# danping/CoSLAM

Measured on AMD Instinct MI355X. Metric: frames/sec for track+local-BA loop, 8 cams 640x480 x 2000 feats (one frame = all 8 cameras), higher is better.
Workload: dtype f32 (KLT, f16 pyramid storage) + f64 (pose, BA)

## Files before the change

coslam_amd/csrc/poseupdate.hip:

```cpp
#include <atomic>
#include <cstdlib>
#include <vector>

#include "cs_common.h"
#include "project_dev.h"
#include "history_view.h"
#include "register_rows_dev.h"
#include "small_ops.h"

#pragma clang fp contract(off)

namespace {

constexpr int PU_MAX_CAMS = 16;
constexpr int PU_MAX_HIST = 512;
constexpr int PU_MAX_STORE = 1 << 16;
constexpr int PU_LPS = 8;

struct PuArgs {
    int nCams, N, nMap, cam0, nCamsRun;
    int gateBlocks, dynBlocksPerCam;
    const int* pointFeat;
    const double* R;
    const double* t;
// ... 302 lines not shown
        double M[3], cov[9];
#pragma unroll
        for (int q = 0; q < 3; ++q) M[q] = A.M[3 * (size_t)p + q];
#pragma unroll
        for (int q = 0; q < 9; ++q) cov[q] = A.cov[9 * (size_t)p + q];
        const int f1 = C.trackSpan[s], f2 = C.trackSpan[N + s];
        const int len = f1 >= 0 ? f2 - f1 + 1 : 0;
        const int depth = len < A.nHist ? len : A.nHist;
        cut = len > A.nHist;
        for (int j = r; j < depth && !fail && !cut; j += MG_LPC) {
            const double* R = mg_pose + 12 * j;
            const double* t = R + 9;
            const int rs = (A.head - j + H) % H;
            const double mx = hXY[(size_t)rs * 2 * N + s], my = hXY[(size_t)rs * 2 * N + N + s];
            fail = mg_term_fails(C.K, R, t, M, cov, A.sigma, mx, my);
        }
    }
    const unsigned long long b = __builtin_amdgcn_ballot_w64(fail);
    if (live && r == 0) {
        const bool anyFail = ((b >> (MG_LPC * g)) & ((1ull << MG_LPC) - 1ull)) != 0ull;
        A.out[(size_t)p * A.nCams + c] = s < 0 ? 255 : (cut ? 2 : (anyFail ? 0 : 1));
    }
}


struct MgCache {
    int slot1;
    int f1;
    int upto;
    int ok;
    double M[3];
    int epoch;
    int pad;
};
static_assert(sizeof(MgCache) == 48, "cs_register_mergability_cache_bytes");
struct MgRunCore {
    MgCore a;
    int W, count, curFrame;
    double tolPix;
    MgCache* cache;
    int epoch, fromMin;
    int* counts;
    const int* list;
    int nList;
    const int* flags;
};
struct MgRunArgs : MgRunCore {
    cs_poseupdate_cam cam[PU_MAX_CAMS];
};
constexpr int MG_GAP_MAX = 2 * MG_LPC;
struct MgMiss {
    int p, s, start, end;
};
template <int NT>
__device__ __forceinline__ void mg_running_rows(const MgRunCore& B, const cs_poseupdate_cam* cams, const int* list, int nList, int c, int bx,
                                                double* mg_pose, MgMiss* missList, int& nMiss) {
    const MgCore& A = B.a;
    const int tid = threadIdx.x, N = A.N, H = A.H, W = B.W;
    if (list && (int)(bx * (NT / MG_LPC)) < nList && list[bx * (NT / MG_LPC)] < 0) return;
    const cs_poseupdate_cam& C = cams[c];
    const double* hR = A.histR + (size_t)c * H * 9;
    const double* hT = A.histT + (size_t)c * H * 3;
    const double* hXY = A.histXY + (size_t)c * H * 2 * N;
    for (int q = tid; q < W * 12; q += NT) {
        const int j = q / 12, e = q - 12 * j, rs = (A.head - j + H) % H;
        mg_pose[q] = e < 9 ? hR[(size_t)rs * 9 + e] : hT[(size_t)rs * 3 + (e - 9)];
    }
    if (tid == 0) nMiss = 0;
    __syncthreads();
    const int lane = tid & 63, r = lane % MG_LPC, g = lane / MG_LPC;
    const unsigned long long gmask = ((1ull << MG_LPC) - 1ull) << (MG_LPC * g);
    const int jj = (bx * NT + tid) / MG_LPC;
    const int p = list ? (jj < nList ? list[jj] : -1) : (jj < A.P ? jj : -1);
    const bool live = p >= 0 && p < A.P;
    int s = live ? A.slot[(size_t)p * A.nCams + c] : -1;
    bool skipped = false;
    if (s >= 0 && B.flags && !(B.flags[(size_t)p * A.nCams + c] & 1)) skipped = true, s = -2;
    bool failW = false, cut = false, tailOK = true, hit = false, listed = false;
    int nTerms = 0;
    if (s >= 0) {
        double M[3], cov[9];
#pragma unroll
        for (int q = 0; q < 3; ++q) M[q] = A.M[3 * (size_t)p + q];
#pragma unroll
        for (int q = 0; q < 9; ++q) cov[q] = A.cov[9 * (size_t)p + q];
        const int f1 = C.trackSpan[s], f2 = C.trackSpan[N + s];
        const int len = f1 >= 0 ? f2 - f1 + 1 : 0;
        const int depth = len < W ? len : W;
        for (int j = r; j < depth && !failW; j += MG_LPC) {
            const double* R = mg_pose + 12 * j;
            const double* t = R + 9;
            const int rs = (A.head - j + H) % H;
            const double mx = hXY[(size_t)rs * 2 * N + s], my = hXY[(size_t)rs * 2 * N + N + s];
            failW = mg_term_fails(C.K, R, t, M, cov, A.sigma, mx, my);
        }
        failW = (__builtin_amdgcn_ballot_w64(failW) & gmask) != 0ull;
        const int end = B.curFrame - W;
        if (len > W) {
            MgCache* E = B.cache + (size_t)p * A.nCams + c;
            const MgCache e = *E;
            const PuProj q0 = pu_project(C.K, mg_pose, mg_pose + 9, M), q1 = pu_project(C.K, mg_pose, mg_pose + 9, e.M);
            const double du = q0.u / q0.w - q1.u / q1.w, dv = q0.v / q0.w - q1.v / q1.w;
            hit = e.slot1 == s + 1 && e.f1 == f1 && e.upto >= f1 - 1 && e.upto <= end && q0.w > 0 && q1.w > 0 &&
                  du * du + dv * dv <= B.tolPix * B.tolPix && (e.epoch == B.epoch || e.upto < B.fromMin);
            const int start = hit ? e.upto + 1 : f1;
            tailOK = hit ? e.ok != 0 : true;
// ... 42 lines not shown
            w.M[0] = M[0], w.M[1] = M[1], w.M[2] = M[2], w.epoch = B.epoch, w.pad = 0;
            B.cache[(size_t)p * A.nCams + c] = w;
        }
    }
    if (live && r == 0 && !listed) A.out[(size_t)p * A.nCams + c] = s == -1 ? 255 : (skipped ? 0 : (cut ? 2 : (failW || !tailOK ? 0 : 1)));
    __syncthreads();
    const int wv = tid >> 6, nM = nMiss;
    for (int k = wv; k < nM; k += NT / 64) {
        const MgMiss m = missList[k];
        double M[3], cov[9];
#pragma unroll
        for (int q = 0; q < 3; ++q) M[q] = A.M[3 * (size_t)m.p + q];
#pragma unroll
        for (int q = 0; q < 9; ++q) cov[q] = A.cov[9 * (size_t)m.p + q];
        bool ok = true;
        for (int f = m.start; f <= m.end && ok; f += 64) {
            bool fail = false;
            const int ff = f + lane;
            if (ff <= m.end) {
                const int j = B.curFrame - ff, rs = ((A.head - j) % H + H) % H;
                double Rt[12];
#pragma unroll
                for (int q = 0; q < 9; ++q) Rt[q] = hR[(size_t)rs * 9 + q];
#pragma unroll
                for (int q = 0; q < 3; ++q) Rt[9 + q] = hT[(size_t)rs * 3 + q];
                const double mx = hXY[(size_t)rs * 2 * N + m.s], my = hXY[(size_t)rs * 2 * N + N + m.s];
                fail = mg_term_fails(C.K, Rt, Rt + 9, M, cov, A.sigma, mx, my);
                ++nTerms;
            }
            if (__builtin_amdgcn_ballot_w64(fail)) ok = false;
        }
        if (lane == 0) {
            MgCache* E = B.cache + (size_t)m.p * A.nCams + c;
            const bool fresh = m.start == C.trackSpan[m.s];
            MgCache w;
            w.slot1 = m.s + 1, w.f1 = C.trackSpan[m.s], w.upto = m.end, w.ok = ok ? 1 : 0;
            w.M[0] = fresh ? M[0] : E->M[0], w.M[1] = fresh ? M[1] : E->M[1], w.M[2] = fresh ? M[2] : E->M[2], w.epoch = B.epoch, w.pad = 0;
            *E = w;
            A.out[(size_t)m.p * A.nCams + c] = ok ? 1 : 0;
        }
    }
    if (B.counts) {
        const unsigned long long bh = __builtin_amdgcn_ballot_w64(hit && r == 0), bw = __builtin_amdgcn_ballot_w64(listed && !hit && r == 0),
                                 bc = __builtin_amdgcn_ballot_w64(cut && r == 0);
        int terms = nTerms;
#pragma unroll
        for (int o = 32; o > 0; o >>= 1) terms += __shfl_xor(terms, o, 64);
        if (lane == 0) {
            if (bh) atomicAdd(B.counts, __popcll(bh));
            if (bw) atomicAdd(B.counts + 1, __popcll(bw));
            if (bc) atomicAdd(B.counts + 2, __popcll(bc));
            if (terms) atomicAdd(B.counts + 3, terms);
        }
    }
}
__global__ __launch_bounds__(256) void k_register_mergability_running(MgRunArgs B) {
    extern __shared__ double mg_pose[];
    __shared__ MgMiss missList[256 / MG_LPC];
    __shared__ int nMiss;
    CS_POSE_STREAM_PRIO();
    mg_running_rows<256>(B, B.cam, B.list, B.nList, B.a.cam0 + blockIdx.y, blockIdx.x, mg_pose, missList, nMiss);
}


struct UpArgs {
    int nCams, N, nMap, H, head, nHist, firstKeyFrame;
    const int* pointFeat;
    const int* lastFrame;
    const unsigned char* isCurrent;
    const double* histXY;
    const double* histR;
    const double* histT;
    double* mapPts;
    double* mapCov;
    const unsigned char* mapFlags;
    double sigma;
    int* counts;
    const double* cen;
    int refine;
    const unsigned char* select;
    const int4* featRef;
    const unsigned char* refStatic;
    const int4* segPool;
    int segCap, curFrame, stored;
    cs_poseupdate_cam cam[PU_MAX_CAMS];
};
constexpr int UP_LPP = 64;

static_assert(UP_LPP == 64 && PU_MAX_CAMS <= UP_LPP, "the covariance tail broadcasts from lane = camera of the point's own wave");

struct UpNormalEq {
    double N[6], g[3];
};
__device__ __forceinline__ void up_add_view(UpNormalEq& E, const double* __restrict__ iK, const double* __restrict__ R,
                                            const double* __restrict__ t, double mx, double my) {
    const double w = (iK[6] * mx + iK[7] * my) + iK[8];
    const double x = ((iK[0] * mx + iK[1] * my) + iK[2]) / w, y = ((iK[3] * mx + iK[4] * my) + iK[5]) / w;
    const double a0[3] = {R[0] - x * R[6], R[1] - x * R[7], R[2] - x * R[8]}, a1[3] = {R[3] - y * R[6], R[4] - y * R[7], R[5] - y * R[8]};
    const double b0 = x * t[2] - t[0], b1 = y * t[2] - t[1];
    E.N[0] = E.N[0] + (a0[0] * a0[0] + a1[0] * a1[0]);
    E.N[1] = E.N[1] + (a0[0] * a0[1] + a1[0] * a1[1]);
    E.N[2] = E.N[2] + (a0[0] * a0[2] + a1[0] * a1[2]);
    E.N[3] = E.N[3] + (a0[1] * a0[1] + a1[1] * a1[1]);
    E.N[4] = E.N[4] + (a0[1] * a0[2] + a1[1] * a1[2]);
    E.N[5] = E.N[5] + (a0[2] * a0[2] + a1[2] * a1[2]);
#pragma unroll
// ... 2013 lines not shown
        }
    }
}

extern "C" int cs_feat_ref_advance_refine_dev(cs_track_history* h, void* hip_stream, const cs_poseupdate_cam* cams, int nMap, const int* d_pointFeat,
                                              int curFrame, cs_feat_ref* d_featRef, unsigned char* d_refStatic, int* d_counts, const int* d_list,
                                              int nList, int advanceAll, unsigned char* d_select, int clearSelect, double* d_mapPts,
                                              double* d_mapCov, double pixelErrVar) {
    if (!h || !cams || nMap < 1 || nList < 1 || !d_pointFeat || !d_featRef || !d_list || !d_select || !d_mapPts || !d_mapCov) {
        cs_set_error("cs_feat_ref_advance_refine_dev: bad arguments");
        return CS_ERR_INVALID;
    }
    if (h->count < 1 || curFrame != h->lastFrame) {
        cs_set_error("cs_feat_ref_advance_refine_dev: the history's newest entry must be frame %d (it holds %d frame(s), the newest %d)", curFrame,
                     h->count, h->lastFrame);
        return CS_ERR_INVALID;
    }
    ArArgs A;
    memset((void*)&A, 0, sizeof(A));
    A.nMap = nMap, A.featRef = (const int4*)d_featRef, A.mapPts = d_mapPts, A.mapCov = d_mapCov, A.sigma = pixelErrVar;
    A.refine = 1, A.select = d_select, A.selectW = d_select, A.clearSelect = clearSelect ? 1 : 0;
    A.segPool = h->segPool, A.segCap = h->segCap, A.curFrame = h->lastFrame, A.stored = h->count < h->H ? h->count : h->H;
    A.nCams = h->nCams, A.N = h->N, A.H = h->H, A.head = h->head, A.nHist = hist_walk(h);
    A.histXY = h->xy, A.histR = h->R, A.histT = h->t, A.cen = h->cen;
    A.F.nCams = h->nCams, A.F.N = h->N, A.F.nMap = nMap, A.F.curFrame = curFrame, A.F.segCap = h->segCap;
    A.F.pointFeat = d_pointFeat, A.F.featRef = (int4*)d_featRef, A.F.refStatic = d_refStatic, A.F.segPool = h->segPool, A.F.segCount = h->segCount;
    A.F.counts = d_counts;
    A.list = d_list, A.nList = nList, A.advAll = advanceAll ? 1 : 0;
    CS_HIP(hipSetDevice(h->device));
    hipStream_t s = (hipStream_t)hip_stream;
    if (nMap > h->aliveCap) {
        if (h->alive) CS_HIP(hipFree(h->alive));
        h->alive = nullptr, h->aliveCap = 0;
        CS_HIP(hipMalloc((void**)&h->alive, (size_t)nMap));
        CS_HIP(hipMemsetAsync(h->alive, 1, (size_t)nMap, s));
        h->aliveCap = nMap;
    }
    A.F.alive = h->alive;
    for (int c = 0; c < h->nCams; ++c) {
        if (!cams[c].K || !cams[c].iK || !cams[c].trackSpan) {
            cs_set_error("cs_feat_ref_advance_refine_dev: null pointer in camera %d (K, iK, trackSpan are read)", c);
            return CS_ERR_INVALID;
        }
        A.cam[c] = cams[c];
    }
    hist_centres(h, s);
    A.blocksA = ((advanceAll ? nMap : nList) + 255) / 256;
    hipLaunchKernelGGL(k_advance_refine, dim3(A.blocksA + (nList + 3) / 4), dim3(256), 0, s, A);
    CS_HIP(hipGetLastError());
    return CS_OK;
}

constexpr int RR_THREADS = 256;
struct RrArgs {
    int nRounds, W, H;
    int* lists;
    int* rvCounts;
    cs_register_pass pass;
    cs_register_cam rcam[RG_MAX_CAMS];
    MgRunCore mg;
    RvArgs rv;
    ArArgs ar;
};
static_assert(sizeof(RrArgs) <= 4096, "k_revisit_rounds: the arguments must fit the kernel-argument segment");
template <int MC>
__global__ __launch_bounds__(RR_THREADS) void k_revisit_rounds(RrArgs A) {
    extern __shared__ double rr_pose[];
    __shared__ MgMiss missList[RR_THREADS / MG_LPC];
    __shared__ int nMiss;
    __shared__ int sCnt[RR_THREADS / 64][5];
    if (rd_ld(A.rvCounts) == 0) return;
    CS_POSE_STREAM_PRIO();
    const int tid = threadIdx.x, lane = tid & 63, wave = tid >> 6, C = A.rv.nCams, cap = A.rv.cap, N = A.rv.N;
    const cs_register_pass& Q = A.pass;
    int cnt[5] = {0, 0, 0, 0, 0};
    for (int r = 0; r < A.nRounds; ++r) {
        const int listed = rd_ld(A.rvCounts + r);
        if (listed == 0) break;
        const int n = listed < cap ? listed : cap;
        const int* list = A.lists + (size_t)r * cap;
        for (int k = wave; k < n * C; k += RR_THREADS / 64) {
            const int row = k / C, c = k - row * C, p = list[row];
            if (p < 0) continue;
            const cs_register_cam& Cm = A.rcam[c];
            const size_t o = (size_t)p * C + c;
            int outSlot = -1, outFlags = 0;
            double m0 = 0, m1 = 0, var[4] = {0, 0, 0, 0}, ivar[4] = {0, 0, 0, 0}, outDist = 0;
            Proj q;
            if (rg_pair_begin(Q, Cm, o, p, A.W, A.H, q, m0, m1, var, ivar, outSlot)) {
                double dMin;
                int iMin;
                rg_pair_scan_wave(Cm, N, lane, m0, m1, ivar, dMin, iMin);
                rg_pair_finish(Q, Cm, p, N, q, m0, m1, dMin, iMin, outSlot, outFlags, outDist);
            }
            if (lane == 0) rg_pair_store(Q, o, outSlot, outFlags, outDist, m0, m1, var);
        }
        __syncthreads();
        const int nB = (n * MG_LPC + RR_THREADS - 1) / RR_THREADS;
        for (int c = 0; c < C; ++c)
            for (int bx = 0; bx < nB; ++bx) {
                mg_running_rows<RR_THREADS>(A.mg, A.ar.cam, list, cap, c, bx, rr_pose, missList, nMiss);
                __syncthreads();
            }
        {
            const bool more = r + 1 < A.nRounds;
            const RvRound Rd{list, A.rvCounts + r, more ? A.lists + (size_t)(r + 1) * cap : nullptr, more ? A.rvCounts + r + 1 : nullptr};
            if (n <= RR_THREADS) {
                rv_decide_rows<MC>(A.rv, Rd);
            } else {
                int* rowCode = (int*)(rr_pose + 12 * (size_t)A.mg.W);
                rv_decide_rows_looped<MC, RR_THREADS>(A.rv, Rd, n, rowCode, rowCode + MC * RV_MAX_ROWS);
            }
        }
        __syncthreads();
        for (int j = tid; j < n; j += RR_THREADS) {
            const int m = list[j];
            if (m >= 0 && m < A.ar.nMap && !A.ar.select[m]) fr_advance_row(A.ar.F, A.ar.cam, m, cnt);
        }
        __syncthreads();
        for (int j = wave; j < n; j += RR_THREADS / 64) {
            const int m = list[j];
            if (m >= 0 && m < A.ar.nMap && A.ar.select[m]) ar_refine_row(A.ar, m, lane, cnt);
        }
        __syncthreads();
    }
    if (A.ar.F.counts) {
#pragma unroll
        for (int k = 0; k < 5; ++k) {
            int v = cnt[k];
#pragma unroll
            for (int o = 32; o > 0; o >>= 1) v += __shfl_xor(v, o, 64);
            if (lane == 0) sCnt[wave][k] = v;
        }
        __syncthreads();
        if (tid < 5) {
            int v = 0;
            for (int w = 0; w < RR_THREADS / 64; ++w) v += sCnt[w][tid];
            if (v) atomicAdd(A.ar.F.counts + tid, v);
        }
    }
}
template <int MC>
static int rr_dynamic_lds_limit(int device, size_t* out) {
    static std::atomic<long long> last{-1};
    const long long c = last.load(std::memory_order_acquire);
    if (c >= 0 && (int)(c >> 32) == device) {
        *out = (size_t)(c & 0xffffffffll);
        return CS_OK;
    }
    hipFuncAttributes fa;
    CS_HIP(hipFuncGetAttributes(&fa, (const void*)k_revisit_rounds<MC>));
    constexpr size_t total = MC == 8 ? 65536 : 163840;
    if (fa.sharedSizeBytes >= total) {
        cs_set_error("k_revisit_rounds<%d>: %zu B of static LDS", MC, (size_t)fa.sharedSizeBytes);
        return CS_ERR_INVALID;
    }
    const size_t dyn = total - fa.sharedSizeBytes;
    if (total > 65536) CS_HIP(hipFuncSetAttribute((const void*)k_revisit_rounds<MC>, hipFuncAttributeMaxDynamicSharedMemorySize, (int)dyn));
    if (device >= 0) last.store(((long long)device << 32) | (long long)dyn, std::memory_order_release);
    *out = dyn;
    return CS_OK;
}

extern "C" int cs_register_revisit_rounds_dev(cs_track_history* h, void* hip_stream, const cs_register_cam* regCams, const cs_poseupdate_cam* cams,
                                              int W, int H, const cs_register_pass* pass, int nMap, int curFrame, int mapBase, int kinds,
                                              double* d_mapPts, double* d_mapCov, double pixelErrVar, double tolPix, void* d_mergeCache,
                                              unsigned char* d_mergeable, int* d_rvLists, int* d_rvCounts, int cap, int nRounds, int* d_visitLoop,
                                              int* d_nextLoop, const unsigned char* d_mapFlags, int* d_pointFeat, int* const* d_slot2map,
                                              unsigned char* d_attached, unsigned char* d_regOut, void* d_decideScratch, const int* d_curList,
                                              const int* d_curCount, int curCap, int* d_rvCnt, cs_feat_ref* d_featRef, unsigned char* d_refStatic,
                                              int* d_frefCounts) {
    if (!h || !regCams || !cams || !pass) {
        cs_set_error("cs_register_revisit_rounds_dev: bad arguments (null history, cameras or pass)");
        return CS_ERR_INVALID;
    }
    const int nCams = h->nCams, N = h->N;
    const cs_register_pass& q = *pass;
// ... 18 lines not shown
        cs_set_error("cs_register_revisit_rounds_dev: the history's newest entry must be frame %d (it holds %d frame(s), the newest %d)", curFrame,
                     h->count, h->lastFrame);
        return CS_ERR_INVALID;
    }
    RrArgs A;
    memset((void*)&A, 0, sizeof(A));
    for (int c = 0; c < nCams; ++c) {
        const cs_register_cam& rc = regCams[c];
        if (!rc.K || !rc.R || !rc.t || !rc.xy || !rc.state || !rc.slot2map) {
            cs_set_error("cs_register_revisit_rounds_dev: null pointer in search camera %d", c);
            return CS_ERR_INVALID;
        }
        if (!cams[c].K || !cams[c].iK || !cams[c].trackSpan) {
            cs_set_error("cs_register_revisit_rounds_dev: null pointer in camera %d (K, iK, trackSpan are read)", c);
            return CS_ERR_INVALID;
        }
        if (!d_slot2map[c]) {
            cs_set_error("cs_register_revisit_rounds_dev: null slot2map of camera %d", c);
            return CS_ERR_INVALID;
        }
        A.rcam[c] = rc;
    }
    A.nRounds = nRounds, A.W = W, A.H = H, A.lists = d_rvLists, A.rvCounts = d_rvCounts;
    A.pass = q;
    A.pass.P = cap, A.pass.list = nullptr;
    MgCore& G = A.mg.a;
    G.cam0 = 0, G.nCams = nCams, G.N = N, G.P = nMap, G.H = h->H, G.head = h->head, G.nHist = hist_walk(h);
    G.sigma = pixelErrVar, G.M = d_mapPts, G.cov = d_mapCov, G.slot = q.slot, G.out = d_mergeable;
    G.histXY = h->xy, G.histR = h->R, G.histT = h->t;
    A.mg.W = hist_walk(h), A.mg.count = h->count, A.mg.curFrame = h->lastFrame, A.mg.epoch = h->tailEpoch, A.mg.fromMin = h->tailFromMin;
    A.mg.tolPix = tolPix, A.mg.cache = (MgCache*)d_mergeCache, A.mg.counts = nullptr, A.mg.flags = q.flags;
    RvArgs& V = A.rv;
    V.nCams = nCams, V.N = N, V.P = nMap, V.cap = cap, V.mapBase = mapBase, V.kinds = kinds, V.nextLoop = d_nextLoop, V.visitLoop = d_visitLoop;
    V.slot = q.slot, V.flags = q.flags, V.mergeable = d_mergeable, V.mapFlags = d_mapFlags, V.pointFeat = d_pointFeat;
    for (int c = 0; c < nCams; ++c) V.slot2map[c] = d_slot2map[c];
    V.attached = d_attached, V.regOut = d_regOut, V.curList = d_curList, V.curCount = d_curCount, V.curCap = curCap, V.counts = d_rvCnt;
    V.nextLoopW = d_nextLoop, V.overflow = d_rvCounts + nRounds;
    V.debug = cs_debug_get(CS_DBG_MERGE_PRINT) == 1;
    int* scr = (int*)d_decideScratch + (size_t)nCams * nMap + nMap;
    for (int k = 0; k < 3; ++k) V.owner[k] = scr, scr += (size_t)nCams * N;
    ArArgs& R = A.ar;
    R.nMap = nMap, R.featRef = (const int4*)d_featRef, R.mapPts = d_mapPts, R.mapCov = d_mapCov, R.sigma = pixelErrVar;
    R.refine = 1, R.select = d_regOut, R.selectW = d_regOut, R.clearSelect = 1;
    R.segPool = h->segPool, R.segCap = h->segCap, R.curFrame = h->lastFrame, R.stored = h->count < h->H ? h->count : h->H;
    R.nCams = nCams, R.N = N, R.H = h->H, R.head = h->head, R.nHist = hist_walk(h);
    R.histXY = h->xy, R.histR = h->R, R.histT = h->t, R.cen = h->cen;
    R.F.nCams = nCams, R.F.N = N, R.F.nMap = nMap, R.F.curFrame = curFrame, R.F.segCap = h->segCap;
    R.F.pointFeat = d_pointFeat, R.F.featRef = (int4*)d_featRef, R.F.refStatic = d_refStatic, R.F.segPool = h->segPool, R.F.segCount = h->segCount;
    R.F.counts = d_frefCounts;
    for (int c = 0; c < nCams; ++c) R.cam[c] = cams[c];
    CS_HIP(hipSetDevice(h->device));
    hipStream_t s = (hipStream_t)hip_stream;
    const int MC = nCams <= 8 ? 8 : RD_MAX_CAMS;
    const size_t lds = sizeof(double) * 12 * (size_t)A.mg.W + (cap > RR_THREADS ? sizeof(int) * (size_t)(MC + 1) * RV_MAX_ROWS : 0);
    size_t ldsMax = 0;
    if (const int rc = MC == 8 ? rr_dynamic_lds_limit<8>(h->device, &ldsMax) : rr_dynamic_lds_limit<RD_MAX_CAMS>(h->device, &ldsMax)) return rc;
    if (lds > ldsMax) {
        cs_set_error("cs_register_revisit_rounds_dev: %zu B of LDS (a history window of %d frames, lists of %d rows, %d cameras) where the "
                     "launch may carry %zu", lds, A.mg.W, cap, nCams, ldsMax);
        return CS_ERR_INVALID;
    }
    if (nMap > h->aliveCap) {
        if (h->alive) CS_HIP(hipFree(h->alive));
        h->alive = nullptr, h->aliveCap = 0;
        CS_HIP(hipMalloc((void**)&h->alive, (size_t)nMap));
        CS_HIP(hipMemsetAsync(h->alive, 1, (size_t)nMap, s));
        h->aliveCap = nMap;
    }
    R.F.alive = h->alive;
    hist_centres(h, s);
    if (MC == 8)
        hipLaunchKernelGGL(k_revisit_rounds<8>, dim3(1), dim3(RR_THREADS), lds, s, A);
    else
        hipLaunchKernelGGL(k_revisit_rounds<RD_MAX_CAMS>, dim3(1), dim3(RR_THREADS), lds, s, A);
    CS_HIP(hipGetLastError());
    return CS_OK;
}

extern "C" int cs_track_history_segments(const cs_track_history* h, cs_feat_seg** d_pool, int* cap, int** d_count) {
    if (!h) {
        cs_set_error("cs_track_history_segments: null handle");
        return CS_ERR_INVALID;
    }
    if (d_pool) *d_pool = (cs_feat_seg*)h->segPool;
    if (cap) *cap = h->segCap;
    if (d_count) *d_count = h->segCount;
    return CS_OK;
}

extern "C" int cs_track_history_segment_counts(const cs_track_history* h, int* counts) {
    if (!h || !counts) {
        cs_set_error("cs_track_history_segment_counts: bad arguments");
        return CS_ERR_INVALID;
    }
    CS_HIP(hipSetDevice(h->device));
    CS_HIP(hipMemcpy(counts, h->segCount, sizeof(int) * h->nCams, hipMemcpyDeviceToHost));
    return CS_OK;
}

extern "C" int cs_track_history_load_segments(cs_track_history* h, const cs_feat_seg* segs, int n) {
    if (!h || n < 0 || n > h->segCap || (n > 0 && !segs)) {
        cs_set_error("cs_track_history_load_segments: bad arguments (at most %d segments per camera)", h ? h->segCap : 0);
        return CS_ERR_INVALID;
    }
    CS_HIP(hipSetDevice(h->device));
    std::vector<int> cnt(h->nCams, n);
    for (int c = 0; c < h->nCams && n > 0; ++c)
        CS_HIP(hipMemcpy(h->segPool + (size_t)c * h->segCap, segs + (size_t)c * n, sizeof(int4) * n, hipMemcpyHostToDevice));
    CS_HIP(hipMemcpy(h->segCount, cnt.data(), sizeof(int) * h->nCams, hipMemcpyHostToDevice));
    return CS_OK;
}

extern "C" int cs_track_history_download_segments(const cs_track_history* h, cs_feat_seg* segs, int n) {
    if (!h || !segs || n < 0 || n > h->segCap) {
        cs_set_error("cs_track_history_download_segments: bad arguments (at most %d segments per camera)", h ? h->segCap : 0);
        return CS_ERR_INVALID;
    }
    CS_HIP(hipSetDevice(h->device));
    for (int c = 0; c < h->nCams && n > 0; ++c)
        CS_HIP(hipMemcpy(segs + (size_t)c * n, h->segPool + (size_t)c * h->segCap, sizeof(int4) * n, hipMemcpyDeviceToHost));
    return CS_OK;
}

namespace {
template <class Args>
void up_set_refs(Args& A, const cs_track_history* h) {
    A.segPool = h->segPool, A.segCap = h->segCap, A.curFrame = h->lastFrame, A.stored = h->count < h->H ? h->count : h->H;
// ... 297 lines not shown
```

coslam_amd/csrc/register_rows_dev.h:

```cpp
#pragma once

#include "cs_common.h"

#include <cfloat>

#pragma clang fp contract(off)

namespace {

constexpr int RG_MAX_CAMS = 16;

struct Proj {
    double u, v, w;
    double KR[9];
};

__device__ __forceinline__ void projection_cov(const Proj& q, const double* __restrict__ cov, double sigma, double var[4]) {
    const double ww = q.w * q.w;
    double J[6], JC[6];
#pragma unroll
    for (int j = 0; j < 3; ++j) {
        J[j] = (q.KR[j] * q.w - q.u * q.KR[6 + j]) / ww;
        J[3 + j] = (q.KR[3 + j] * q.w - q.v * q.KR[6 + j]) / ww;
    }
// ... 30 lines not shown
    const double X = ((R[0] * M[0] + R[1] * M[1]) + R[2] * M[2]) + t[0];
    const double Y = ((R[3] * M[0] + R[4] * M[1]) + R[5] * M[2]) + t[1];
    const double Z = ((R[6] * M[0] + R[7] * M[1]) + R[8] * M[2]) + t[2];
    if (Z < 0.0) {
        outSlot = -2;
        return false;
    }
    q.u = (K[0] * X + K[1] * Y) + K[2] * Z;
    q.v = (K[3] * X + K[4] * Y) + K[5] * Z;
    q.w = (K[6] * X + K[7] * Y) + K[8] * Z;
    m0 = q.u / q.w;
    m1 = q.v / q.w;
    if (m0 < 0 || m0 >= (double)W || m1 < 0 || m1 >= (double)H) {
        outSlot = -3;
        return false;
    }
#pragma unroll
    for (int i = 0; i < 3; ++i)
#pragma unroll
        for (int j = 0; j < 3; ++j) q.KR[3 * i + j] = (K[3 * i] * R[j] + K[3 * i + 1] * R[3 + j]) + K[3 * i + 2] * R[6 + j];
    projection_cov(q, Q.cov + 9 * (size_t)p, Q.sigmaSearch, var);
    mat22_inv(var, ivar);
    const bool dynPt = Q.mapFlags && (Q.mapFlags[p] & (CS_MAP_DYNAMIC | CS_MAP_FALSE | CS_MAP_UNCERTAIN)) == CS_MAP_DYNAMIC;
    const double sc = 1 / (dynPt ? Q.maxDistDynamic : Q.maxDist);
#pragma unroll
    for (int k = 0; k < 4; ++k) ivar[k] = ivar[k] * sc;
    return true;
}
__device__ __forceinline__ void rg_pair_finish(const cs_register_pass& Q, const cs_register_cam& C, int p, int N, const Proj& q, double m0,
                                               double m1, double dMin, int iMin, int& outSlot, int& outFlags, double& outDist) {
    if (iMin == 0x7fffffff) {
        outSlot = -4;
        return;
    }
    outSlot = iMin;
    outDist = dMin;
    if (C.slot2map[iMin] < 0) outFlags |= 1;
    if (C.isDynamic ? C.isDynamic[iMin] != 0 : (C.isStatic && C.isStatic[iMin] == 0)) outFlags |= 2;
    double v2[4], iv[4];
    projection_cov(q, Q.cov + 9 * (size_t)p, Q.sigmaMerge, v2);
    mat22_inv(v2, iv);
    if (!(maha_dist2(m0, m1, C.xy[iMin], C.xy[N + iMin], iv) > 1.0)) outFlags |= 4;
}
__device__ __forceinline__ void rg_pair_store(const cs_register_pass& Q, size_t o, int outSlot, int outFlags, double outDist, double m0, double m1,
                                              const double var[4]) {
    Q.slot[o] = outSlot;
    Q.flags[o] = outFlags;
    Q.dist[o] = outDist;
    Q.m[2 * o] = m0;
    Q.m[2 * o + 1] = m1;
#pragma unroll
    for (int k = 0; k < 4; ++k) Q.var[4 * o + k] = var[k];
}
__device__ __forceinline__ void rg_pair_scan_wave(const cs_register_cam& C, int N, int lane, double m0, double m1, const double ivar[4],
                                                  double& dMin, int& iMin) {
    dMin = DBL_MAX, iMin = 0x7fffffff;
    const double* __restrict__ xs = C.xy;
    const double* __restrict__ ys = C.xy + N;
    const int* __restrict__ st = C.state;
    for (int i = lane; i < N; i += 64) {
        const int s = st[i];
        if (s == 0 || s == 1) {
            const double d = maha_dist2(m0, m1, xs[i], ys[i], ivar);
            if (d < dMin) dMin = d, iMin = i;
        }
    }
#pragma unroll
    for (int off = 32; off > 0; off >>= 1) {
        const double d2 = __shfl_xor(dMin, off, 64);
        const int i2 = __shfl_xor(iMin, off, 64);
        if (d2 < dMin || (d2 == dMin && i2 < iMin)) dMin = d2, iMin = i2;
    }
}

constexpr int RD_MAX_CAMS = 16;
constexpr int RD_INIT_MAPPED = 1 << 29, RD_CAN_MERGE = 1 << 28, RD_FEAT = (1 << 28) - 1;
constexpr int RD_INF = 0x7fffffff;
__device__ __forceinline__ int rd_ld(const int* p) { return __hip_atomic_load(p, __ATOMIC_RELAXED, __HIP_MEMORY_SCOPE_AGENT); }
__device__ __forceinline__ void rd_st(int* p, int v) { __hip_atomic_store(p, v, __ATOMIC_RELAXED, __HIP_MEMORY_SCOPE_AGENT); }

struct RvArgs {
    int nCams, N, P, cap, mapBase, kinds;
    const int* list;
    const int* nextLoop;
    int* visitLoop;
    const int* slot;
    const int* flags;
    const unsigned char* mergeable;
    const unsigned char* mapFlags;
    int* pointFeat;
    int* slot2map[RD_MAX_CAMS];
    unsigned char* attached;
    unsigned char* regOut;
    int* owner[3];
    const int* curList;
    const int* curCount;
    int curCap;
    int* counts;
    const int* listCount;
    int* nextList;
    int* nextCount;
    int* nextLoopW;
    int* overflow;
    int debug;
};
constexpr int RV_MAX_ROWS = 1024;
struct RvRound {
    const int* list;
    const int* listCount;
    int* nextList;
    int* nextCount;
};
__device__ __forceinline__ RvRound rv_round_of(const RvArgs& A) { return RvRound{A.list, A.listCount, A.nextList, A.nextCount}; }
__device__ __forceinline__ int* rv_owner(const RvArgs& A, int k) {
    const int r = k % 3;
    return r == 0 ? A.owner[0] : (r == 1 ? A.owner[1] : A.owner[2]);
}
template <int MC>
__device__ __forceinline__ void rv_row_build(const RvArgs& A, int p, int (&code)[MC], int& base, int& nConf) {
    const int C = A.nCams;
    int kind = -1;
    base = -1;
#pragma unroll
    for (int i = 0; i < MC; ++i) code[i] = -1;
    int pfv[MC], slv[MC], flv[MC], own[MC];
    unsigned char mgv[MC];
// ... 99 lines not shown
            }
        }
    }
    if (reg) {
        ++nReg;
        const int last = A.nextLoop[p];
        A.regOut[p] = 1, A.visitLoop[p] = last;
        if (Rd.nextList) {
            int b = -1;
            for (int c = C - 1; c > last; --c)
                if (A.pointFeat[(size_t)p * C + c] >= 0) b = c;
            if (b >= 0) {
                const int q = atomicAdd(Rd.nextCount, 1);
                if (q < A.cap) Rd.nextList[q] = p, A.nextLoopW[p] = b;
                else if (A.overflow) atomicAdd(A.overflow, 1);
            }
        }
    }
}
template <int MC>
__device__ __forceinline__ void rv_conflicts_of(const RvArgs& A, int q, const int (&qs)[MC], const RvAttached& S, int nA, int& nConf) {
    const int C = A.nCams;
    bool any = false;
    for (int a = 0; a < nA && !any; ++a) {
        const int i = S.cam[a], sl = S.sl[a];
#pragma unroll
        for (int t = 0; t < MC; ++t) any |= t == i && qs[t] == sl;
    }
    if (!any) return;
    int qp[MC];
    unsigned qatt = 0;
#pragma unroll
    for (int i = 0; i < MC; ++i) {
        const size_t kq = (size_t)q * C + (i < C ? i : 0);
        qp[i] = A.pointFeat[kq];
        if (i < C && A.attached[kq]) qatt |= 1u << i;
    }
    int lq = -1;
#pragma unroll
    for (int i = MC - 1; i >= 0; --i)
        if (i < C && qp[i] >= 0 && !((qatt >> i) & 1u)) lq = i;
    if (lq < 0) return;
    for (int a = 0; a < nA; ++a) {
        const int i = S.cam[a], sl = S.sl[a];
        int qsi = -1, qpi = 0;
#pragma unroll
        for (int t = 0; t < MC; ++t)
            if (t == i) qsi = qs[t], qpi = qp[t];
        if (qsi != sl || qpi >= 0) continue;
        if ((lq * A.P + q) * C + i <= S.key[a]) continue;
        if ((qatt >> (i + 1)) != 0u) ++nConf;
    }
}
template <int MC>
__device__ __forceinline__ void rv_decide_rows(const RvArgs& A, const RvRound& Rd) {
    __shared__ int sChanged;
    __shared__ RvAttached sAtt;
    const int j = threadIdx.x, C = A.nCams;
    const long long tD0 = A.debug ? wall_clock64() : 0;
    long long tD1 = 0, tD2 = 0, tD3 = 0;
    const int p = j < A.cap ? Rd.list[j] : -1;
    int code[MC], base = -1, nConf = 0;
    if (j == 0) sAtt.n = 0;
    const int nCurPre = *A.curCount < A.curCap ? *A.curCount : A.curCap;
    int preQ[2], preS[2][MC];
#pragma unroll
    for (int u = 0; u < 2; ++u) {
        const int e = j + u * (int)blockDim.x;
        preQ[u] = e < nCurPre ? A.curList[e] : -1;
        if (preQ[u] >= A.P) preQ[u] = -1;
#pragma unroll
        for (int i = 0; i < MC; ++i) preS[u][i] = preQ[u] >= 0 ? A.slot[(size_t)preQ[u] * C + (i < C ? i : 0)] : -1;
    }
    rv_row_build<MC>(A, p, code, base, nConf);
    __syncthreads();
    if (A.debug) tD1 = wall_clock64();
    int k = 0;
    const int* fin = A.owner[0];
    bool settled = false;
    for (; k < 32; ++k) {
        const int* prev = rv_owner(A, k);
        int* next = rv_owner(A, k + 1);
        int* clear = rv_owner(A, k + 2);
        if (j == 0) sChanged = 0;
        rv_row_clear<MC>(code, base, clear);
        __syncthreads();
        rv_row_claim<MC>(code, base, prev, next);
        __syncthreads();
        if (rv_row_changed<MC>(code, base, prev, next)) sChanged = 1;
        __syncthreads();
        fin = next;
        const int chg = sChanged;
        __syncthreads();
        if (!chg) {
            settled = true;
            break;
        }
    }
    if (A.debug) tD2 = wall_clock64();
    int nAtt = 0, nReg = 0;
    rv_row_attach<MC>(A, Rd, p, code, base, fin, sAtt, nAtt, nReg);
    __syncthreads();
    if (A.debug) tD3 = wall_clock64();
    const int nA = sAtt.n < 256 ? sAtt.n : 256;
    if (nA > 0) {
        const int nCur = nCurPre;
        for (int e = j, u = 0; e < nCur; e += (int)blockDim.x, ++u) {
            const int q = u == 0 ? preQ[0] : (u == 1 ? preQ[1] : A.curList[e]);
            if (q < 0 || q >= A.P) continue;
            int qs[MC];
#pragma unroll
            for (int i = 0; i < MC; ++i) qs[i] = u == 0 ? preS[0][i] : (u == 1 ? preS[1][i] : A.slot[(size_t)q * C + (i < C ? i : 0)]);
            rv_conflicts_of<MC>(A, q, qs, sAtt, nA, nConf);
        }
    }
    if (A.debug && j == 0)
        printf("k_revisit_decide: rows %d; build %lld us, %d sweeps %lld us, attach %lld us (%d attached), scan %lld us\n", Rd.listCount ? *Rd.listCount : -1,
               (tD1 - tD0) / 100, k + 1, (tD2 - tD1) / 100, (tD3 - tD2) / 100, nA, (wall_clock64() - tD3) / 100);
    if (A.counts) {
        if (nAtt) atomicAdd(A.counts, nAtt);
        if (nReg) atomicAdd(A.counts + 1, nReg);
        if (nConf) atomicAdd(A.counts + 2, nConf);
        if (j == 0 && !settled) atomicAdd(A.counts + 3, 1);
    }
}
template <int MC, int NT>
__device__ __forceinline__ void rv_decide_rows_looped(const RvArgs& A, const RvRound& Rd, int n, int* rowCode, int* rowBase) {
    __shared__ int sChanged;
    __shared__ RvAttached sAtt;
    const int tid = threadIdx.x, C = A.nCams;
    int code[MC], base, nConf = 0;
    if (tid == 0) sAtt.n = 0;
    for (int j = tid; j < n; j += NT) {
        rv_row_build<MC>(A, Rd.list[j], code, base, nConf);
        rowBase[j] = base;
#pragma unroll
        for (int i = 0; i < MC; ++i) rowCode[i * RV_MAX_ROWS + j] = code[i];
    }
    __syncthreads();
    int k = 0;
    const int* fin = A.owner[0];
    bool settled = false;
    for (; k < 32; ++k) {
        const int* prev = rv_owner(A, k);
        int* next = rv_owner(A, k + 1);
        int* clear = rv_owner(A, k + 2);
        if (tid == 0) sChanged = 0;
        for (int j = tid; j < n; j += NT) {
#pragma unroll
            for (int i = 0; i < MC; ++i) code[i] = rowCode[i * RV_MAX_ROWS + j];
            rv_row_clear<MC>(code, rowBase[j], clear);
        }
        __syncthreads();
        for (int j = tid; j < n; j += NT) {
#pragma unroll
            for (int i = 0; i < MC; ++i) code[i] = rowCode[i * RV_MAX_ROWS + j];
            rv_row_claim<MC>(code, rowBase[j], prev, next);
        }
        __syncthreads();
        int ch = 0;
        for (int j = tid; j < n; j += NT) {
#pragma unroll
            for (int i = 0; i < MC; ++i) code[i] = rowCode[i * RV_MAX_ROWS + j];
            ch |= rv_row_changed<MC>(code, rowBase[j], prev, next);
        }
        if (ch) sChanged = 1;
        __syncthreads();
        fin = next;
        const int chg = sChanged;
        __syncthreads();
        if (!chg) {
            settled = true;
            break;
        }
    }
    int nAtt = 0, nReg = 0;
    for (int j = tid; j < n; j += NT) {
#pragma unroll
        for (int i = 0; i < MC; ++i) code[i] = rowCode[i * RV_MAX_ROWS + j];
        rv_row_attach<MC>(A, Rd, Rd.list[j], code, rowBase[j], fin, sAtt, nAtt, nReg);
    }
    __syncthreads();
    const int nA = sAtt.n < 256 ? sAtt.n : 256;
    if (nA > 0) {
        const int nCur = *A.curCount < A.curCap ? *A.curCount : A.curCap;
        for (int e = tid; e < nCur; e += NT) {
            const int q = A.curList[e];
            if (q < 0 || q >= A.P) continue;
            int qs[MC];
#pragma unroll
            for (int i = 0; i < MC; ++i) qs[i] = A.slot[(size_t)q * C + (i < C ? i : 0)];
            rv_conflicts_of<MC>(A, q, qs, sAtt, nA, nConf);
        }
    }
    if (A.debug && tid == 0) printf("k_revisit_rounds: rows %d in turns of %d; %d sweeps, %d attached\n", n, NT, k + 1, nA);
    if (A.counts) {
        if (nAtt) atomicAdd(A.counts, nAtt);
        if (nReg) atomicAdd(A.counts + 1, nReg);
        if (nConf) atomicAdd(A.counts + 2, nConf);
        if (tid == 0 && !settled) atomicAdd(A.counts + 3, 1);
    }
}

}
```

Baseline: 2016.

## Restructure revisit-rounds kernel: per-thread pair setup, all-camera mergability pairs, batched scans

In the single-block revisit-rounds kernel, pair setup now runs one pair per thread, with results staged in LDS before the waves scan. Mergability is evaluated across all cameras in one pass, with an adaptive lanes-per-candidate count and the pose windows of all cameras preloaded into LDS, replacing the earlier per-camera block loop. The feature scan and window checks batch their loads to raise memory-level parallelism. The change also adds debug phase timers and a print kernel, and it costs more LDS plus extra block-wide barriers.

Measured after the change: 2012. Within noise of the previous version (-0.2%).

```diff
diff --git a/coslam_amd/csrc/poseupdate.hip b/coslam_amd/csrc/poseupdate.hip
--- a/coslam_amd/csrc/poseupdate.hip
+++ b/coslam_amd/csrc/poseupdate.hip
@@ -378,6 +378,98 @@
 struct MgMiss {
     int p, s, start, end;
 };
+
+__device__ __forceinline__ void mg_candidate_tail(int LPC, const MgRunCore& B, const cs_poseupdate_cam& C, const double* pose0, const double* hR,
+                                                  const double* hT, const double* hXY, MgCache* E, const MgCache& e, int s, int r,
+                                                  unsigned long long gmask, const double (&M)[3], const double (&cov)[9], int f1, bool failW,
+                                                  bool& cut, bool& tailOK, bool& hit, bool& listed, int& start, int& end, int& nTerms) {
+    const MgCore& A = B.a;
+    const int N = A.N, H = A.H, W = B.W;
+    end = B.curFrame - W;
+    const PuProj q0 = pu_project(C.K, pose0, pose0 + 9, M), q1 = pu_project(C.K, pose0, pose0 + 9, e.M);
+    const double du = q0.u / q0.w - q1.u / q1.w, dv = q0.v / q0.w - q1.v / q1.w;
+    hit = e.slot1 == s + 1 && e.f1 == f1 && e.upto >= f1 - 1 && e.upto <= end && q0.w > 0 && q1.w > 0 &&
+          du * du + dv * dv <= B.tolPix * B.tolPix && (e.epoch == B.epoch || e.upto < B.fromMin);
+    start = hit ? e.upto + 1 : f1;
+    tailOK = hit ? e.ok != 0 : true;
+    const bool shortGap = end - start + 1 <= MG_GAP_MAX;
+    bool wrote = false;
+    if (start > end) {
+        wrote = hit;
+    } else if (!tailOK) {
+        wrote = true;
+    } else if (B.curFrame - start >= B.count) {
+        cut = !failW;
+    } else if (shortGap && (hit || !failW)) {
+        for (int f = start; f <= end && tailOK; f += LPC) {
+            bool fail = false;
+            const int ff = f + r;
+            if (ff <= end) {
+                const int j = B.curFrame - ff, rs = ((A.head - j) % H + H) % H;
+                double Rt[12];
+#pragma unroll
+                for (int q = 0; q < 9; ++q) Rt[q] = hR[(size_t)rs * 9 + q];
+#pragma unroll
+                for (int q = 0; q < 3; ++q) Rt[9 + q] = hT[(size_t)rs * 3 + q];
+                const double mx = hXY[(size_t)rs * 2 * N + s], my = hXY[(size_t)rs * 2 * N + N + s];
+                fail = mg_term_fails(C.K, Rt, Rt + 9, M, cov, A.sigma, mx, my);
+                ++nTerms;
+            }
+            if (__builtin_amdgcn_ballot_w64(fail) & gmask) tailOK = false;
+        }
+        wrote = true;
+    } else if (!failW) {
+        listed = true;
+    }
+    if (wrote && r == 0) {
+        MgCache w;
+        w.slot1 = s + 1, w.f1 = f1, w.upto = end, w.ok = tailOK ? 1 : 0;
+        w.M[0] = hit ? e.M[0] : M[0], w.M[1] = hit ? e.M[1] : M[1], w.M[2] = hit ? e.M[2] : M[2], w.epoch = B.epoch, w.pad = 0;
+        *E = w;
+    }
+}
+__device__ __forceinline__ void mg_candidate_no_tail(const MgRunCore& B, MgCache* E, int s, int f1, const double (&M)[3]) {
+    MgCache w;
+    w.slot1 = s + 1, w.f1 = f1, w.upto = f1 - 1, w.ok = 1;
+    w.M[0] = M[0], w.M[1] = M[1], w.M[2] = M[2], w.epoch = B.epoch, w.pad = 0;
+    *E = w;
+}
+__device__ __forceinline__ void mg_tail_wave(const MgRunCore& B, const cs_poseupdate_cam& C, int c, const double* hR, const double* hT,
+                                             const double* hXY, int p, int s, int start, int end, int lane, int& nTerms) {
+    const MgCore& A = B.a;
+    const int N = A.N, H = A.H;
+    double M[3], cov[9];
+#pragma unroll
+    for (int q = 0; q < 3; ++q) M[q] = A.M[3 * (size_t)p + q];
+#pragma unroll
+    for (int q = 0; q < 9; ++q) cov[q] = A.cov[9 * (size_t)p + q];
+    bool ok = true;
+    for (int f = start; f <= end && ok; f += 64) {
+        bool fail = false;
+        const int ff = f + lane;
+        if (ff <= end) {
+            const int j = B.curFrame - ff, rs = ((A.head - j) % H + H) % H;
+            double Rt[12];
+#pragma unroll
+            for (int q = 0; q < 9; ++q) Rt[q] = hR[(size_t)rs * 9 + q];
+#pragma unroll
+            for (int q = 0; q < 3; ++q) Rt[9 + q] = hT[(size_t)rs * 3 + q];
+            const double mx = hXY[(size_t)rs * 2 * N + s], my = hXY[(size_t)rs * 2 * N + N + s];
+            fail = mg_term_fails(C.K, Rt, Rt + 9, M, cov, A.sigma, mx, my);
+            ++nTerms;
+        }
+        if (__builtin_amdgcn_ballot_w64(fail)) ok = false;
+    }
+    if (lane == 0) {
+        MgCache* E = B.cache + (size_t)p * A.nCams + c;
+        const bool fresh = start == C.trackSpan[s];
+        MgCache w;
+        w.slot1 = s + 1, w.f1 = C.trackSpan[s], w.upto = end, w.ok = ok ? 1 : 0;
+        w.M[0] = fresh ? M[0] : E->M[0], w.M[1] = fresh ? M[1] : E->M[1], w.M[2] = fresh ? M[2] : E->M[2], w.epoch = B.epoch, w.pad = 0;
+        *E = w;
+        A.out[(size_t)p * A.nCams + c] = ok ? 1 : 0;
+    }
+}
 template <int NT>
 __device__ __forceinline__ void mg_running_rows(const MgRunCore& B, const cs_poseupdate_cam* cams, const int* list, int nList, int c, int bx,
                                                 double* mg_pose, MgMiss* missList, int& nMiss) {
@@ -526,6 +618,82 @@
             if (bc) atomicAdd(B.counts + 2, __popcll(bc));
             if (terms) atomicAdd(B.counts + 3, terms);
         }
+    }
+}
+struct MgMissCam {
+    MgMiss m;
+    int c;
+};
+template <int NT>
+__device__ __forceinline__ void mg_running_pairs(int LPC, const MgRunCore& B, const cs_poseupdate_cam* cams, const int* list, int n,
+                                                 const double* pose, MgMissCam* missList, int& nMiss) {
+    constexpr int MG_WIN_BATCH = 8;
+    const MgCore& A = B.a;
+    const int tid = threadIdx.x, N = A.N, H = A.H, W = B.W, nC = A.nCams;
+    const int lane = tid & 63, r = lane % LPC, g = lane / LPC;
+    const unsigned long long gmask = ((1ull << LPC) - 1ull) << (LPC * g);
+    for (int k0 = 0; k0 < n * nC; k0 += NT / LPC) {
+        if (tid == 0) nMiss = 0;
+        __syncthreads();
+        const int kk = k0 + tid / LPC, row = kk / nC, c = kk - row * nC;
+        const int p = kk < n * nC ? list[row] : -1;
+        const bool live = p >= 0 && p < A.P;
+        const cs_poseupdate_cam& C = cams[c];
+        const double* hR = A.histR + (size_t)c * H * 9;
+        const double* hT = A.histT + (size_t)c * H * 3;
+        const double* hXY = A.histXY + (size_t)c * H * 2 * N;
+        const double* mg_pose = pose + (size_t)c * W * 12;
+        int s = live ? A.slot[(size_t)p * nC + c] : -1;
+        bool skipped = false;
+        if (s >= 0 && B.flags && !(B.flags[(size_t)p * nC + c] & 1)) skipped = true, s = -2;
+        bool failW = false, cut = false, tailOK = true, hit = false, listed = false;
+        int nTerms = 0;
+        if (s >= 0) {
+            MgCache* E = B.cache + (size_t)p * nC + c;
+            const MgCache e = *E;
+            double M[3], cov[9];
+#pragma unroll
+            for (int q = 0; q < 3; ++q) M[q] = A.M[3 * (size_t)p + q];
+#pragma unroll
+            for (int q = 0; q < 9; ++q) cov[q] = A.cov[9 * (size_t)p + q];
+            const int f1 = C.trackSpan[s], f2 = C.trackSpan[N + s];
+            const int len = f1 >= 0 ? f2 - f1 + 1 : 0;
+            const int depth = len < W ? len : W;
+            for (int j0 = r; j0 < depth && !failW; j0 += LPC * MG_WIN_BATCH) {
+                double mx[MG_WIN_BATCH], my[MG_WIN_BATCH];
+#pragma unroll
+                for (int u = 0; u < MG_WIN_BATCH; ++u) {
+                    const int j = j0 + LPC * u < depth ? j0 + LPC * u : j0, rs = (A.head - j + H) % H;
+                    mx[u] = hXY[(size_t)rs * 2 * N + s], my[u] = hXY[(size_t)rs * 2 * N + N + s];
+                }
+#pragma unroll
+                for (int u = 0; u < MG_WIN_BATCH; ++u) {
+                    const int j = j0 + LPC * u;
+                    if (j < depth && !failW) failW = mg_term_fails(C.K, mg_pose + 12 * j, mg_pose + 12 * j + 9, M, cov, A.sigma, mx[u], my[u]);
+                }
+            }
+            failW = (__builtin_amdgcn_ballot_w64(failW) & gmask) != 0ull;
+            if (len > W) {
+                int start, end;
+                mg_candidate_tail(LPC, B, C, mg_pose, hR, hT, hXY, E, e, s, r, gmask, M, cov, f1, failW, cut, tailOK, hit, listed, start, end, nTerms);
+                if (listed && r == 0) {
+                    const int k = atomicAdd(&nMiss, 1);
+                    missList[k] = MgMissCam{MgMiss{p, s, start, end}, c};
+                }
+            } else if (len > 0 && r == 0) {
+                mg_candidate_no_tail(B, E, s, f1, M);
+            }
+        }
+        if (live && r == 0 && !listed) A.out[(size_t)p * nC + c] = s == -1 ? 255 : (skipped ? 0 : (cut ? 2 : (failW || !tailOK ? 0 : 1)));
+        __syncthreads();
+        const int wv = __builtin_amdgcn_readfirstlane(tid >> 6), nM = nMiss;
+        for (int k = wv; k < nM; k += NT / 64) {
+            const MgMiss m = missList[k].m;
+            const int cm = missList[k].c;
+            mg_tail_wave(B, cams[cm], cm, A.histR + (size_t)cm * H * 9, A.histT + (size_t)cm * H * 3, A.histXY + (size_t)cm * H * 2 * N, m.p, m.s,
+                         m.start, m.end, lane, nTerms);
+        }
+        if (k0 + NT / LPC < n * nC) __syncthreads();
     }
 }
 __global__ __launch_bounds__(256) void k_register_mergability_running(MgRunArgs B) {
@@ -2645,8 +2813,22 @@
 }
 
 constexpr int RR_THREADS = 256;
+__device__ int g_rrPhase[8][12];
+__device__ int g_rrRounds;
+__global__ void k_revisit_rounds_print() {
+    if (threadIdx.x != 0) return;
+    for (int r = 0; r < g_rrRounds; ++r) {
+        const int* q = g_rrPhase[r];
+        printf("k_revisit_rounds: round %d rows %d; search %.2f us, mergability %.2f us, walks %.2f us (build %.2f, %d sweeps %.2f, attach %.2f "
+               "(%d attached), scan %.2f), advance %.2f us, refine %.2f us\n",
+               r, q[0], q[1] / 100.0, q[2] / 100.0, q[3] / 100.0, q[6] / 100.0, q[10], q[7] / 100.0, q[8] / 100.0, q[11], q[9] / 100.0, q[4] / 100.0,
+               q[5] / 100.0);
+    }
+    g_rrRounds = 0;
+}
 struct RrArgs {
     int nRounds, W, H;
+    int mgPairs;
     int* lists;
     int* rvCounts;
     cs_register_pass pass;
@@ -2659,63 +2841,105 @@
 template <int MC>
 __global__ __launch_bounds__(RR_THREADS) void k_revisit_rounds(RrArgs A) {
     extern __shared__ double rr_pose[];
-    __shared__ MgMiss missList[RR_THREADS / MG_LPC];
+    __shared__ MgMissCam missCam[RR_THREADS / MG_LPC];
     __shared__ int nMiss;
     __shared__ int sCnt[RR_THREADS / 64][5];
     if (rd_ld(A.rvCounts) == 0) return;
     CS_POSE_STREAM_PRIO();
-    const int tid = threadIdx.x, lane = tid & 63, wave = tid >> 6, C = A.rv.nCams, cap = A.rv.cap, N = A.rv.N;
+    const int tid = threadIdx.x, lane = tid & 63, wave = __builtin_amdgcn_readfirstlane(tid >> 6), C = A.rv.nCams, cap = A.rv.cap, N = A.rv.N;
     const cs_register_pass& Q = A.pass;
+    RgTurn& T = *(RgTurn*)rr_pose;
     int cnt[5] = {0, 0, 0, 0, 0};
     for (int r = 0; r < A.nRounds; ++r) {
         const int listed = rd_ld(A.rvCounts + r);
         if (listed == 0) break;
         const int n = listed < cap ? listed : cap;
         const int* list = A.lists + (size_t)r * cap;
-        for (int k = wave; k < n * C; k += RR_THREADS / 64) {
-            const int row = k / C, c = k - row * C, p = list[row];
-            if (p < 0) continue;
-            const cs_register_cam& Cm = A.rcam[c];
-            const size_t o = (size_t)p * C + c;
+        long long tP[6] = {0, 0, 0, 0, 0, 0};
+        if (A.rv.debug) tP[0] = wall_clock64();
+        for (int k0 = 0; k0 < n * C; k0 += RG_TURN_PAIRS) {
+            const int k = k0 + tid, nT = n * C - k0 < RG_TURN_PAIRS ? n * C - k0 : RG_TURN_PAIRS;
+            const int row = k / C, c = k - row * C, p = tid < nT ? list[row] : -1;
+            const size_t o = (size_t)(p < 0 ? 0 : p) * C + c;
             int outSlot = -1, outFlags = 0;
             double m0 = 0, m1 = 0, var[4] = {0, 0, 0, 0}, ivar[4] = {0, 0, 0, 0}, outDist = 0;
             Proj q;
-            if (rg_pair_begin(Q, Cm, o, p, A.W, A.H, q, m0, m1, var, ivar, outSlot)) {
+            const bool scan = p >= 0 && rg_pair_begin(Q, A.rcam[c], o, p, A.W, A.H, q, m0, m1, var, ivar, outSlot);
+            if (tid < nT) {
+                T.scan[tid] = scan ? 1 : 0;
+                if (scan) {
+                    T.m0[tid] = m0, T.m1[tid] = m1;
+#pragma unroll
+                    for (int e = 0; e < 4; ++e) T.ivar[e][tid] = ivar[e];
+                }
+            }
+            __syncthreads();
+            for (int j = wave; j < nT; j += RR_THREADS / 64) {
+                if (!T.scan[j]) continue;
+                const int cj = (k0 + j) % C;
+                const double iv[4] = {T.ivar[0][j], T.ivar[1][j], T.ivar[2][j], T.ivar[3][j]};
                 double dMin;
                 int iMin;
-                rg_pair_scan_wave(Cm, N, lane, m0, m1, ivar, dMin, iMin);
-                rg_pair_finish(Q, Cm, p, N, q, m0, m1, dMin, iMin, outSlot, outFlags, outDist);
+                rg_pair_scan_wave(A.rcam[cj], N, lane, T.m0[j], T.m1[j], iv, dMin, iMin);
+                if (lane == 0) T.dMin[j] = dMin, T.iMin[j] = iMin;
             }
-            if (lane == 0) rg_pair_store(Q, o, outSlot, outFlags, outDist, m0, m1, var);
+            __syncthreads();
+            if (p >= 0) {
+                if (scan) rg_pair_finish(Q, A.rcam[c], p, N, q, m0, m1, T.dMin[tid], T.iMin[tid], outSlot, outFlags, outDist);
+                rg_pair_store(Q, o, outSlot, outFlags, outDist, m0, m1, var);
+            }
+            __syncthreads();
         }
         __syncthreads();
-        const int nB = (n * MG_LPC + RR_THREADS - 1) / RR_THREADS;
-        for (int c = 0; c < C; ++c)
-            for (int bx = 0; bx < nB; ++bx) {
-                mg_running_rows<RR_THREADS>(A.mg, A.ar.cam, list, cap, c, bx, rr_pose, missList, nMiss);
-                __syncthreads();
+        if (A.rv.debug) tP[1] = wall_clock64();
+        if (A.mgPairs) {
+            const int Wd = A.mg.W, Hh = A.mg.a.H;
+            for (int q = tid; q < C * Wd * 12; q += RR_THREADS) {
+                const int c = q / (Wd * 12), q1 = q - c * (Wd * 12), j = q1 / 12, e = q1 - 12 * j, rs = (A.mg.a.head - j + Hh) % Hh;
+                rr_pose[q] = e < 9 ? A.mg.a.histR[((size_t)c * Hh + rs) * 9 + e] : A.mg.a.histT[((size_t)c * Hh + rs) * 3 + (e - 9)];
             }
+            mg_running_pairs<RR_THREADS>(n * C * 32 <= RR_THREADS ? 32 : (n * C * 16 <= RR_THREADS ? 16 : MG_LPC), A.mg, A.ar.cam, list, n, rr_pose,
+                                         missCam, nMiss);
+            __syncthreads();
+        } else {
+            const int nB = (n * MG_LPC + RR_THREADS - 1) / RR_THREADS;
+            for (int c = 0; c < C; ++c)
+                for (int bx = 0; bx < nB; ++bx) {
+                    mg_running_rows<RR_THREADS>(A.mg, A.ar.cam, list, cap, c, bx, rr_pose, (MgMiss*)missCam, nMiss);
+                    __syncthreads();
+                }
+        }
+        if (A.rv.debug) tP[2] = wall_clock64();
         {
             const bool more = r + 1 < A.nRounds;
             const RvRound Rd{list, A.rvCounts + r, more ? A.lists + (size_t)(r + 1) * cap : nullptr, more ? A.rvCounts + r + 1 : nullptr};
             if (n <= RR_THREADS) {
-                rv_decide_rows<MC>(A.rv, Rd);
+                rv_decide_rows<MC, false>(A.rv, Rd, &g_rrPhase[r][6]);
             } else {
                 int* rowCode = (int*)(rr_pose + 12 * (size_t)A.mg.W);
-                rv_decide_rows_looped<MC, RR_THREADS>(A.rv, Rd, n, rowCode, rowCode + MC * RV_MAX_ROWS);
+                rv_decide_rows_looped<MC, RR_THREADS>(A.rv, Rd, n, rowCode, rowCode + MC * RV_MAX_ROWS, &g_rrPhase[r][6]);
             }
         }
         __syncthreads();
+        if (A.rv.debug) tP[3] = wall_clock64();
         for (int j = tid; j < n; j += RR_THREADS) {
             const int m = list[j];
             if (m >= 0 && m < A.ar.nMap && !A.ar.select[m]) fr_advance_row(A.ar.F, A.ar.cam, m, cnt);
         }
         __syncthreads();
+        if (A.rv.debug) tP[4] = wall_clock64();
         for (int j = wave; j < n; j += RR_THREADS / 64) {
             const int m = list[j];
             if (m >= 0 && m < A.ar.nMap && A.ar.select[m]) ar_refine_row(A.ar, m, lane, cnt);
         }
         __syncthreads();
+        if (A.rv.debug && tid == 0) {
+            tP[5] = wall_clock64();
+            g_rrPhase[r][0] = n;
+#pragma unroll
+            for (int k = 0; k < 5; ++k) g_rrPhase[r][1 + k] = (int)(tP[k + 1] - tP[k]);
+            g_rrRounds = r + 1;
+        }
     }
     if (A.ar.F.counts) {
 #pragma unroll
@@ -2840,9 +3064,13 @@
     CS_HIP(hipSetDevice(h->device));
     hipStream_t s = (hipStream_t)hip_stream;
     const int MC = nCams <= 8 ? 8 : RD_MAX_CAMS;
-    const size_t lds = sizeof(double) * 12 * (size_t)A.mg.W + (cap > RR_THREADS ? sizeof(int) * (size_t)(MC + 1) * RV_MAX_ROWS : 0);
+    size_t lds = sizeof(double) * 12 * (size_t)A.mg.W + (cap > RR_THREADS ? sizeof(int) * (size_t)(MC + 1) * RV_MAX_ROWS : 0);
+    if (lds < sizeof(RgTurn)) lds = sizeof(RgTurn);
     size_t ldsMax = 0;
     if (const int rc = MC == 8 ? rr_dynamic_lds_limit<8>(h->device, &ldsMax) : rr_dynamic_lds_limit<RD_MAX_CAMS>(h->device, &ldsMax)) return rc;
+    const size_t ldsPairs = sizeof(double) * 12 * (size_t)A.mg.W * nCams;
+    A.mgPairs = ldsPairs <= ldsMax ? 1 : 0;
+    if (A.mgPairs && lds < ldsPairs) lds = ldsPairs;
     if (lds > ldsMax) {
         cs_set_error("cs_register_revisit_rounds_dev: %zu B of LDS (a history window of %d frames, lists of %d rows, %d cameras) where the "
                      "launch may carry %zu", lds, A.mg.W, cap, nCams, ldsMax);
@@ -2861,6 +3089,7 @@
         hipLaunchKernelGGL(k_revisit_rounds<8>, dim3(1), dim3(RR_THREADS), lds, s, A);
     else
         hipLaunchKernelGGL(k_revisit_rounds<RD_MAX_CAMS>, dim3(1), dim3(RR_THREADS), lds, s, A);
+    if (V.debug) hipLaunchKernelGGL(k_revisit_rounds_print, dim3(1), dim3(1), 0, s);
     CS_HIP(hipGetLastError());
     return CS_OK;
 }
diff --git a/coslam_amd/csrc/register_rows_dev.h b/coslam_amd/csrc/register_rows_dev.h
--- a/coslam_amd/csrc/register_rows_dev.h
+++ b/coslam_amd/csrc/register_rows_dev.h
@@ -106,17 +106,27 @@
 #pragma unroll
     for (int k = 0; k < 4; ++k) Q.var[4 * o + k] = var[k];
 }
+constexpr int RG_SCAN_BATCH = 8;
 __device__ __forceinline__ void rg_pair_scan_wave(const cs_register_cam& C, int N, int lane, double m0, double m1, const double ivar[4],
                                                   double& dMin, int& iMin) {
     dMin = DBL_MAX, iMin = 0x7fffffff;
     const double* __restrict__ xs = C.xy;
     const double* __restrict__ ys = C.xy + N;
     const int* __restrict__ st = C.state;
-    for (int i = lane; i < N; i += 64) {
-        const int s = st[i];
-        if (s == 0 || s == 1) {
-            const double d = maha_dist2(m0, m1, xs[i], ys[i], ivar);
-            if (d < dMin) dMin = d, iMin = i;
+    for (int i0 = lane; i0 < N; i0 += 64 * RG_SCAN_BATCH) {
+        int sv[RG_SCAN_BATCH];
+        double xv[RG_SCAN_BATCH], yv[RG_SCAN_BATCH];
+#pragma unroll
+        for (int u = 0; u < RG_SCAN_BATCH; ++u) {
+            const int i = i0 + 64 * u, ii = i < N ? i : i0;
+            sv[u] = st[ii], xv[u] = xs[ii], yv[u] = ys[ii];
+        }
+#pragma unroll
+        for (int u = 0; u < RG_SCAN_BATCH; ++u) {
+            const int i = i0 + 64 * u;
+            const double d = maha_dist2(m0, m1, xv[u], yv[u], ivar);
+            const bool less = (i < N) & ((sv[u] == 0) | (sv[u] == 1)) & (d < dMin);
+            dMin = less ? d : dMin, iMin = less ? i : iMin;
         }
     }
 #pragma unroll
@@ -126,6 +136,12 @@
         if (d2 < dMin || (d2 == dMin && i2 < iMin)) dMin = d2, iMin = i2;
     }
 }
+constexpr int RG_TURN_PAIRS = 256;
+struct RgTurn {
+    double m0[RG_TURN_PAIRS], m1[RG_TURN_PAIRS], ivar[4][RG_TURN_PAIRS], dMin[RG_TURN_PAIRS];
+    int iMin[RG_TURN_PAIRS];
+    int scan[RG_TURN_PAIRS];
+};
 
 constexpr int RD_MAX_CAMS = 16;
 constexpr int RD_INIT_MAPPED = 1 << 29, RD_CAN_MERGE = 1 << 28, RD_FEAT = (1 << 28) - 1;
@@ -331,8 +347,8 @@
         if ((qatt >> (i + 1)) != 0u) ++nConf;
     }
 }
-template <int MC>
-__device__ __forceinline__ void rv_decide_rows(const RvArgs& A, const RvRound& Rd) {
+template <int MC, bool PRINT = true>
+__device__ __forceinline__ void rv_decide_rows(const RvArgs& A, const RvRound& Rd, int* walkTicks = nullptr) {
     __shared__ int sChanged;
     __shared__ RvAttached sAtt;
     const int j = threadIdx.x, C = A.nCams;
@@ -393,9 +409,14 @@
             rv_conflicts_of<MC>(A, q, qs, sAtt, nA, nConf);
         }
     }
-    if (A.debug && j == 0)
-        printf("k_revisit_decide: rows %d; build %lld us, %d sweeps %lld us, attach %lld us (%d attached), scan %lld us\n", Rd.listCount ? *Rd.listCount : -1,
-               (tD1 - tD0) / 100, k + 1, (tD2 - tD1) / 100, (tD3 - tD2) / 100, nA, (wall_clock64() - tD3) / 100);
+    if constexpr (PRINT) {
+        if (A.debug && j == 0)
+            printf("k_revisit_decide: rows %d; build %lld us, %d sweeps %lld us, attach %lld us (%d attached), scan %lld us\n", Rd.listCount ? *Rd.listCount : -1,
+                   (tD1 - tD0) / 100, k + 1, (tD2 - tD1) / 100, (tD3 - tD2) / 100, nA, (wall_clock64() - tD3) / 100);
+    } else if (A.debug && j == 0) {
+        walkTicks[0] = (int)(tD1 - tD0), walkTicks[1] = (int)(tD2 - tD1), walkTicks[2] = (int)(tD3 - tD2), walkTicks[3] = (int)(wall_clock64() - tD3);
+        walkTicks[4] = k + 1, walkTicks[5] = nA;
+    }
     if (A.counts) {
         if (nAtt) atomicAdd(A.counts, nAtt);
         if (nReg) atomicAdd(A.counts + 1, nReg);
@@ -404,7 +425,7 @@
     }
 }
 template <int MC, int NT>
-__device__ __forceinline__ void rv_decide_rows_looped(const RvArgs& A, const RvRound& Rd, int n, int* rowCode, int* rowBase) {
+__device__ __forceinline__ void rv_decide_rows_looped(const RvArgs& A, const RvRound& Rd, int n, int* rowCode, int* rowBase, int* walkTicks) {
     __shared__ int sChanged;
     __shared__ RvAttached sAtt;
     const int tid = threadIdx.x, C = A.nCams;
@@ -472,7 +493,7 @@
             rv_conflicts_of<MC>(A, q, qs, sAtt, nA, nConf);
         }
     }
-    if (A.debug && tid == 0) printf("k_revisit_rounds: rows %d in turns of %d; %d sweeps, %d attached\n", n, NT, k + 1, nA);
+    if (A.debug && tid == 0) walkTicks[0] = walkTicks[1] = walkTicks[2] = walkTicks[3] = -1, walkTicks[4] = k + 1, walkTicks[5] = nA;
     if (A.counts) {
         if (nAtt) atomicAdd(A.counts, nAtt);
         if (nReg) atomicAdd(A.counts + 1, nReg);
```
